# WilliamYi96/HGR-Net

Measured on AMD Instinct MI355X. Metric: images/sec over 21K-class hierarchy, batch 512; hit@1 parity vs reference, higher is better.
Workload: dtype f16

## Files before the change

hgr-net_amd/_lib.py:

```python
from __future__ import annotations

import ctypes as C
import os
from pathlib import Path

import torch

_HERE = Path(__file__).resolve().parent
LIB_PATH = Path(os.environ.get("HGR_LIB", _HERE / "lib" / "libhgr.so"))

HGR_BF16, HGR_F16 = 0, 1
EPI_NONE, EPI_BIAS, EPI_BIAS_QUICKGELU, EPI_BIAS_RESIDUAL, EPI_BIAS_RELU, EPI_BIAS_ADD16_RELU, EPI_ACCUM, EPI_QGELU_GRAD16 = 0, 1, 2, 3, 4, 5, 6, 7

_p, _i, _l, _f = C.c_void_p, C.c_int, C.c_int64, C.c_float

SIGNATURES = {
    "hgr_gemm_nt": [_p, _l, _p, _l, _p, _l, _p, _p, _l, _i, _i, _i, _i, _i, _i, _p],
    "hgr_gemm_set_tile": [_i],
    "hgr_gemm_set_tail": [_i, _i],
    "hgr_gemm_set_persist": [_i],
    "hgr_gemm_set_ws": [_i],
    "hgr_gemm_set_p8": [_i],
    "hgr_im2col_patches": [_p, _p, _i, _i, _i, _i, _i, _p],
    "hgr_im2col_patches_ex": [_p, _p, _i, _i, _i, _i, _i, _i, _i, _p],
# ... 52 lines not shown
    "hgr_avgpool2_bwd_nhwc": [_p, _p, _i, _i, _i, _i, _i, _p],
    "hgr_attnpool_tokens_bwd": [_p, _p, _i, _i, _i, _i, _p],
    "hgr_im2col3x3_t": [_p, _p, _i, _i, _i, _i, _l, _i, _p],
    "hgr_bn_fold": [_p, _p, _p, _p, _p, _f, _p, _p, _i, _i, _i, _i, _i, _p],
    "hgr_bn_unfold_grad": [_p, _l, _p, _p, _p, _p, _p, _f, _p, _p, _p, _i, _i, _i, _p],
    "hgr_csr_group_aggregate": [_p, _l, _p, _p, _p, _p, _i, _p, _p, _p, _p, _i, _p, _p, _p, _p, _i, _p, _p, _l, _i, _f, _i, _p],
    "hgr_gemm_nt_res_stats": [_p, _l, _p, _l, _p, _p, _l, _p, _p, _i, _i, _i, _i, _p],
    "hgr_vit_head": [_p, _p, _l, _l, _p, _p, _f, _p, _p, _i, _i, _i, _i, _p],
    "hgr_gemm_nt_res_stats_guard": [_p, _l, _p, _l, _p, _p, _l, _p, _p, _f, _p, _i, _i, _i, _i, _p],
    "hgr_gemm_nt_ln": [_p, _l, _p, _l, _p, _l, _p, _p, _p, _f, _i, _i, _i, _i, _i, _p],
    "hgr_gemm_nt_ln_mha": [_p, _l, _p, _l, _p, _p, _p, _f, _p, _l, _i, _i, _i, _i, _i, _p],
    "hgr_gemm_nt_bias_gelu_dual": [_p, _l, _p, _l, _p, _l, _p, _l, _p, _i, _i, _i, _i, _p],
    "hgr_gemm_nt_qgelu_grad_colsum": [_p, _l, _p, _l, _p, _l, _p, _l, _p, _i, _i, _i, _i, _p],
    "hgr_vit_embed_ln_stats": [_p, _p, _p, _p, _p, _p, _p, _p, _i, _i, _i, _f, _i, _p],
    "hgr_row_stats16": [_p, _p, _p, _p, _i, _i, _i, _p],
    "hgr_pair_rows_f32": [_p, _p, _p, _i, _i, _l, _p, _i, _p],
    "hgr_logits_eval_workspace_bytes": [_i, _i],
    "hgr_logits_eval": [_p, _p, _i, _i, _i, _p, _p, _p, _i, _p, _p, _i, _p, _i, _i, _p, _p, _p, _p, _i, _p],
    "hgr_logits_eval_tile_stage": [_p, _p, _i, _i, _i, _p, _p, _p, _i, _p, _p, _i, _p, _i, _i, _p, _p, _p, _p, _i, _p],
    "hgr_logits_eval_row_stage": [_p, _p, _i, _i, _i, _p, _p, _p, _i, _p, _p, _i, _p, _i, _i, _p, _p, _p, _p, _i, _p],
    "hgr_comm_unique_id": [_p],
    "hgr_comm_init": [_i, _i, _p],
    "hgr_comm_destroy": [],
    "hgr_comm_rank": [],
    "hgr_comm_world": [],
    "hgr_allreduce": [_p, _p, _l, _i, _i, _p],
    "hgr_allgather": [_p, _p, _l, _i, _p],
    "hgr_broadcast": [_p, _l, _i, _i, _p],
    "hgr_adamw": [_p, _p, _p, _p, _l, _f, _f, _f, _f, _f, _i, _p, _f, _f, _p],
}
# ... 55 lines not shown
```

hgr-net_amd/clip/model.py:

```python
from __future__ import annotations

import os
from collections import OrderedDict
from typing import Dict, Optional, Tuple, Union

import numpy as np
import torch
from torch import nn

from .. import ops
from .._lib import (EPI_BIAS, EPI_BIAS_ADD16_RELU, EPI_BIAS_QUICKGELU, EPI_BIAS_RELU, EPI_BIAS_RESIDUAL, EPI_NONE,
                    HgrError)


class QuickGELU(nn.Module):
    """Placeholder so ``mlp`` keeps the reference's child names (c_fc, gelu, c_proj); the activation
    itself is fused into the c_fc GEMM epilogue (HGR_EPI_BIAS_QUICKGELU)."""


class ResidualAttentionBlock(nn.Module):
    def __init__(self, d_model: int, n_head: int):
        super().__init__()
        self.attn = nn.MultiheadAttention(d_model, n_head)
        self.ln_1 = nn.LayerNorm(d_model)
# ... 111 lines not shown
        t = self._b.get("const." + name)
        if t is None:
            t = self._b["const." + name] = build()
            self.epoch += 1
        return t

    def get(self, name: str, shape, dtype, device) -> torch.Tensor:
        n = int(np.prod(shape))
        t = self._b.get(name)
        if t is None or t.numel() < n or t.dtype != dtype or t.device != device:
            t = torch.empty(n, dtype=dtype, device=device)
            self._b[name] = t
            self.epoch += 1
        return t[:n].view(*shape)


IMG_STREAMS = max(1, int(os.environ.get("HGR_IMG_STREAMS", "1")))
IMG_STREAMS_MIN_ROWS = 8192
CLS_LAST = os.environ.get("HGR_CLS_LAST", "1") != "0"
LN_FUSED = os.environ.get("HGR_LN_FUSED", "1") != "0"
QKV_MHA = os.environ.get("HGR_QKV_MHA", "1") != "0"


def ln_fusable(w: int, m: int = 0) -> bool:
    return LN_FUSED and w % 128 == 0 and m * 4 * w * 2 < 2 ** 32


def _run_blocks(x: Optional[torch.Tensor], blocks, heads: int, b: int, l: int, causal: bool, dt: torch.dtype, ws: _Workspace, tag: str,
                taps: Optional[dict] = None, tap_prefix: str = "", pair=None, stats: Optional[torch.Tensor] = None,
                flag: Optional[torch.Tensor] = None, cls_only_last: bool = False):
    m, w = (pair[0] if pair is not None else x).shape
    dev = (pair[0] if pair is not None else x).device
    qkv = ws.get(tag + ".qkv", (m, 3 * w), dt, dev)
    att = ws.get(tag + ".att", (m, w), dt, dev)
    u16 = ws.get(tag + ".u16", (m, 4 * w), dt, dev)
    if pair is not None:
        xh, xl = pair
        for i, k in enumerate(blocks):
            last_cls = cls_only_last and i == len(blocks) - 1 and l > 1 and 3 * w * l < (1 << 23)
            fused_attn = QKV_MHA and not last_cls and ops.ln_mha_ok(w, l, m, xh.stride(0))
            if last_cls:
                ch, cl = xh.view(b, l, w)[:, 0, :], xl.view(b, l, w)[:, 0, :]
                ops.gemm_nt_ln(xh, k.wf_in[w:], qkv[:, w:], k.s_in[w:], k.c_in[w:], stats, k.eps1, tag="kv")
                ops.split_point("class_token_tail")
                st_q = ws.get(tag + ".stats_q", (b, w // 64, 2), torch.float32, dev)
                idx = ws.const(f"cls_rows.{b}.{l}", lambda: (torch.arange(b, dtype=torch.int32, device=dev) * l).contiguous())
                ops.rows_gather(stats.view(b * l, -1), idx, st_q.view(b, -1))
                ops.gemm_nt_ln(ch, k.wf_in[:w], qkv.view(b, l, 3 * w)[:, 0, :w], k.s_in[:w], k.c_in[:w], st_q, k.eps1, tag="q_cls")
            elif fused_attn:
                ops.gemm_nt_ln_mha(xh, k.wf_in, att, k.s_in, k.c_in, stats, b, l, heads, causal, k.eps1)
            else:
                ops.gemm_nt_ln(xh, k.wf_in, qkv, k.s_in, k.c_in, stats, k.eps1, tag="qkv")
            if not fused_attn:
                ops.mha(qkv, att, b, l, heads, causal, q_rows=1 if last_cls else 0)
            if last_cls:
                ca = att.view(b, l, w)[:, 0, :]
                st_c = ws.get(tag + ".stats_cls", (b, w // 64, 2), torch.float32, dev)
                u_c = ws.get(tag + ".u16_cls", (b, 4 * w), dt, dev)
                ops.gemm_nt_res_stats(ca, k.w_out, ch, cl, k.b_out, st_c, tag="out_cls", flag=flag)
# ... 304 lines not shown
        return have[:n]

    def _vit_forward(self, image: torch.Tensor, p: dict, out: torch.Tensor, tag: str, taps: Optional[dict], u8: bool) -> bool:
        v = self.visual
        dt, ws, dev = self.image_dtype, self._ws, image.device
        b, r = image.shape[0], v.input_resolution
        ps = v.patch_size
        g = r // ps
        gg, l, w = g * g, g * g + 1, v.conv1.weight.shape[0]
        patches = ws.get(tag + ".patches", (b * gg, p["kp"]), dt, dev)
        if u8:
            ops.im2col_patches_u8(image, patches, ps)
        else:
            ops.im2col_patches(image, patches, ps)
        pe = ws.get(tag + ".pe", (b * gg, w), torch.float32, dev)
        ops.gemm_nt(patches, p["conv_w_nhwc"] if u8 else p["conv_w"], pe, tag="patch")
        cls16 = ws.get(tag + ".cls16", (b, w), dt, dev)
        fused = ln_fusable(w, b * l) and "v" not in self._ln_off
        if fused:
            xh = ws.get(tag + ".xh", (b * l, w), dt, dev)
            xl = ws.get(tag + ".xl", (b * l, w), ops.PAIR_LO, dev)
            stats = ws.get(tag + ".stats", (b * l, w // 64, 2), torch.float32, dev)
            ops.vit_embed_ln_stats(pe, p["cls"], p["pos"], p["ln_pre"][0], p["ln_pre"][1], xh, xl, stats, b, gg)
            if taps is not None:
                taps["visual.ln_pre"] = ops.pair_value(xh, xl).view(b, l, w)
            _run_blocks(None, p["vblocks"], w // 64, b, l, False, dt, ws, tag, taps, "visual.transformer", (xh, xl), stats, self._ln_flag("v", dev),
                        cls_only_last=taps is None and CLS_LAST)
            if w <= 1920 and w % 32 == 0 and v.output_dim % 4 == 0:
                ops.vit_head(xh, xl, l, p["ln_post"][0], p["ln_post"][1], float(v.ln_post.eps), p["proj_t"], out)
                return fused
            cls32 = ws.get(tag + ".cls32", (b, w), torch.float32, dev)
            ops.pair_rows_f32(xh, xl, cls32, row_mul=l)
            ops.layernorm(cls32, p["ln_post"][0], p["ln_post"][1], cls16, rows=b)
        else:
            x = ws.get(tag + ".x", (b * l, w), torch.float32, dev)
            ops.vit_embed_ln(pe, p["cls"], p["pos"], p["ln_pre"][0], p["ln_pre"][1], x, b, gg)
            if taps is not None:
                taps["visual.ln_pre"] = x.view(b, l, w).clone()
# ... 86 lines not shown
```

hgr-net_amd/csrc/hgr_common.h:

```cpp
#pragma once
#include <hip/hip_runtime.h>
#include <stdint.h>
#include <stdio.h>
#include <stdarg.h>
#include <stdlib.h>

#include "../../include/hgr.h"

#define HGR_WAVE 64

#ifdef HGR_LAB
#define HGR_LAB_ON(expr) (expr)
static inline int hgr_lab_env(const char *name) { const char *e = getenv(name); return e ? atoi(e) : 0; }
#else
#define HGR_LAB_ON(expr) false
static inline int hgr_lab_env(const char *) { return 0; }
#endif

typedef __attribute__((ext_vector_type(8))) __bf16 bf16x8;
typedef __attribute__((ext_vector_type(8))) _Float16 f16x8;
typedef __attribute__((ext_vector_type(4))) __bf16 bf16x4;
typedef __attribute__((ext_vector_type(4))) _Float16 f16x4;
typedef __attribute__((ext_vector_type(4))) float f32x4;
typedef __attribute__((ext_vector_type(16))) float f32x16;
// ... 126 lines not shown
}
__device__ __forceinline__ float wave_max(float v) {
#pragma unroll
    for (int o = 32; o > 0; o >>= 1) v = fmaxf(v, __shfl_xor(v, o));
    return v;
}

__device__ __forceinline__ float row16_sum(float v) {
    v += __builtin_bit_cast(float, __builtin_amdgcn_update_dpp(0, __builtin_bit_cast(int, v), 0xB1, 0xF, 0xF, true));
    v += __builtin_bit_cast(float, __builtin_amdgcn_update_dpp(0, __builtin_bit_cast(int, v), 0x4E, 0xF, 0xF, true));
    v += __builtin_bit_cast(float, __builtin_amdgcn_update_dpp(0, __builtin_bit_cast(int, v), 0x141, 0xF, 0xF, true));
    v += __builtin_bit_cast(float, __builtin_amdgcn_update_dpp(0, __builtin_bit_cast(int, v), 0x140, 0xF, 0xF, true));
    return v;
}

int hgr_set_error(int code, const char *fmt, ...);

#define HGR_REQUIRE(cond, ...)                                            \
    do {                                                                  \
        if (!(cond)) return hgr_set_error(HGR_EINVAL, __VA_ARGS__);       \
    } while (0)

#define HGR_CHECK_LAUNCH(name)                                                                      \
    do {                                                                                            \
        hipError_t e__ = hipGetLastError();                                                         \
        if (e__ != hipSuccess) return hgr_set_error(HGR_ELAUNCH, "%s: %s", name, hipGetErrorString(e__)); \
    } while (0)

static inline bool hgr_aligned(const void *p, size_t a) { return (reinterpret_cast<uintptr_t>(p) % a) == 0; }
```

hgr-net_amd/csrc/hgr_gemm.hip:

```cpp
#include "hgr_gemm_common.h"

using namespace hgr_gemm;

int hgr_conv3x3_c32_launch(const void *x, const void *w, const float *bias, void *out, int B, int H, int W, int Cout, int Kp,
                           int dtype, int relu, void *stream, int pool, int C);

namespace {
constexpr int BM = 128, BN = 128;

int duo_group_env() {
    static int g = -1;
    if (g < 0) { const char *e = getenv("HGR_GEMM_GROUP"); g = e ? atoi(e) : 0; if (g < 0) g = 0; }
    return g;
}
int duo_group() { return duo_group_env() ? duo_group_env() : 4; }
int duo_group_for(int tiles_n) { return duo_group_env() ? duo_group_env() : (tiles_n <= 8 ? 1 : 4); }
int duo_dbg() {
    static int d = -1;
    if (d < 0) d = hgr_lab_env("HGR_GEMM_DBG");
    return d;
}

struct DuoPlan { int big_panels, nbig, tiles_m_half, grid; };
int tail_env = -2, pb_env = -2;
// ... 180 lines not shown
        a.res = nullptr; a.ldr = 0; a.M = M; a.N = N; a.K = K;
        a.m_fastest = ((int64_t)N * K > (int64_t)M * K) ? 1 : 0;
        a.vec_ok = 1; a.dbg = dbg; a.kc = 0; a.csplit = 0; a.group = duo_group();
        launch_ws(a, dtype, WS_PLAIN, epilogue == HGR_EPI_BIAS_RELU ? 2 : 0, epilogue != HGR_EPI_NONE, s);
    }
    else if (duo_ok && (force == 2 || (force == 0 && tduo >= 256 && duo_fits))) launch_d();
    else if (force == 128 || K < 128) launch(0, M, false);
    else if (epi_has_idn16(epilogue) && force != 256) launch(0, M, false);
    else if (force == 256) launch(0, M, true);
    else if (cost_split < cost_big && cost_split < cost_small) { launch(0, m1, true); launch(m1, M - m1, false); }
    else launch(0, M, cost_big <= cost_small && t256 >= 128);
    HGR_CHECK_LAUNCH("hgr_gemm_nt");
    return HGR_OK;
}

static int conv3x3_launch(const void *x, const void *w, const float *bias, void *out,
                          int B, int H, int W, int C, int Cout, int stride, int Kp, int dtype, bool relu, void *stream) {
    HGR_REQUIRE(x && w && out && (bias || !relu), "hgr_conv3x3_nhwc: null operand");
    HGR_REQUIRE(B >= 1 && H >= 1 && W >= 1 && Cout >= 1 && (stride == 1 || stride == 2), "hgr_conv3x3_nhwc: bad geometry B=%d H=%d W=%d Cout=%d stride=%d", B, H, W, Cout, stride);
    HGR_REQUIRE(C >= 8 && C % 8 == 0 && C <= 16384, "hgr_conv3x3_nhwc: C=%d must be a multiple of 8 in [8, 16384]", C);
    HGR_REQUIRE(Kp >= 9 * C && Kp % BK == 0, "hgr_conv3x3_nhwc: Kp=%d must be >= 9*C and a multiple of %d", Kp, BK);
    HGR_REQUIRE(hgr_aligned(x, 16) && hgr_aligned(w, 16) && hgr_aligned(out, 8) && (!bias || hgr_aligned(bias, 16)) && Cout % 4 == 0, "hgr_conv3x3_nhwc: misaligned operand / Cout %% 4 != 0");
    HGR_REQUIRE(dtype == HGR_BF16 || dtype == HGR_F16, "hgr_conv3x3_nhwc: bad dtype %d", dtype);
    static int direct_env = -1;
    if (direct_env < 0) { const char *e = getenv("HGR_CONV_DIRECT"); direct_env = e ? atoi(e) : 1; }
    if (direct_env && C == 32 && stride == 1 && (Cout == 32 || Cout == 64) && Kp >= 288 && hgr_aligned(out, 16))
        return hgr_conv3x3_c32_launch(x, w, bias, out, B, H, W, Cout, Kp, dtype, relu ? 1 : 0, stream, 0, 32);
    if (direct_env && C == 64 && Cout == 64 && stride == 1 && Kp >= 576 && hgr_aligned(out, 16) && (int64_t)B * H * W >= 4096)
        return hgr_conv3x3_c32_launch(x, w, bias, out, B, H, W, Cout, Kp, dtype, relu ? 1 : 0, stream, 0, 64);
    const int Ho = (H + 2 - 3) / stride + 1, Wo = (W + 2 - 3) / stride + 1;
// ... 241 lines not shown
```

hgr-net_amd/csrc/hgr_gemm_common.h:

```cpp
#pragma once
#include "hgr_common.h"
#include <stdlib.h>
#include <type_traits>

namespace hgr_gemm {

constexpr int BK = 64;

struct GemmArgs {
    const char *A; int64_t lda;
    const char *W; int64_t ldw;
    void *C; int64_t ldc;
    const float *bias;
    const float *res; int64_t ldr;
    int M, N, K;
    int tiles_m, tiles_n;
    int m_fastest;
    int vec_ok;
    int dbg;
    int cH, cW, cC, cStride, cHo, cWo;
    unsigned cMagic;
    int cUni;
    int kc; int64_t csplit;
    float *ln_stats; int ln_slots; float ln_eps;
    void *ln_xh, *ln_xl; int64_t ln_ldx;
    const float *ln_s, *ln_c;
    unsigned *ln_flag; float ln_guard;
    int group;
    int nbig, big_panels, tiles_m_half;
    float *colsum = nullptr; int colsum_units = 0;
    int total = 0;
};


static __device__ __attribute__((aligned(16))) unsigned int hgr_zero_page[4] = {0u, 0u, 0u, 0u};

__device__ __forceinline__ float quick_gelu(float v) {
    return v * __builtin_amdgcn_rcpf(1.0f + __builtin_amdgcn_exp2f(-1.702f * 1.4426950408889634f * v));
}


template <int DT> __device__ __forceinline__ typename T16<DT>::elem quick_gelu16(float v) {
    return mul16<DT>(v, __builtin_amdgcn_rcpf(1.0f + __builtin_amdgcn_exp2f(-1.702f * 1.4426950408889634f * v)));
}
template <int DT> __device__ __forceinline__ typename T16<DT>::elem quick_gelu_train16(float x) {
// ... 224 lines not shown
```

hgr-net_amd/csrc/hgr_gemm_duo.hip:

```cpp
#include "hgr_gemm_common.h"

namespace hgr_gemm {

#ifndef HGR_PAIR_V2
#define HGR_PAIR_V2 1
#endif
constexpr int NTD = 256;
constexpr int DUO_A0 = 0, DUO_A1 = 32768, DUO_W0 = 65536, DUO_W1 = 73728, DUO_LDS = 81920;

__device__ __forceinline__ void store16_sc1(void *ptr, u32x4 v) {
    asm volatile("global_store_dwordx4 %0, %1, off sc1\n\ts_nop 1" ::"v"(ptr), "v"(v) : "memory");
}

template <int DT, int EPI, bool OUT32, int LN, int MH, bool CONV = false>
__device__ __forceinline__ void duo_tile(const GemmArgs &p, char *smem, const int m0, const int n0) {
    typedef typename T16<DT>::vec8 vec8;
    typedef typename T16<DT>::elem E;
    constexpr int WR = 64 * MH;
    int tid = threadIdx.x;
    if (LN == 1) asm volatile("" : "+v"(tid));
    const int lane = tid & 63;
    const int wave = __builtin_amdgcn_readfirstlane(tid >> 6);
    const int wm = wave >> 1, wn = wave & 1;
    const int r = lane & 15, g = lane >> 4;
// ... 786 lines not shown
    for (int a = 0; a < MH; ++a)
#pragma unroll
    for (int i = 0; i < 4; ++i) {
        const int m = m0 + wm * WR + a * 64 + i * 16 + r;
        if (m >= p.M) continue;
#pragma unroll
        for (int b = 0; b < 2; ++b)
#pragma unroll
        for (int j = 0; j < 2; ++j) {
            const int n = n0 + wn * 64 + b * 32 + j * 16 + g * 4;
            if (n < p.N) store_quad<DT, EPI, OUT32>(p, acc[a][b][i][j], m, n);
        }
    }
}

template <int DT, int EPI, bool OUT32, int LN = 0, bool CONV = false>
__global__ __launch_bounds__(NTD, 2) void gemm_nt_duo(GemmArgs p) {
    if (p.kc) {
        const int sp = blockIdx.y;
        p.A += (int64_t)sp * p.kc * 2; p.W += (int64_t)sp * p.kc * 2;
        p.C = (char *)p.C + (int64_t)sp * p.csplit * 4;
        p.K = min(p.kc, p.K - sp * p.kc);
    }
    __shared__ __attribute__((aligned(1024))) char smem[DUO_LDS];
    constexpr bool PERSIST = LN == 1;
    const int total = PERSIST && p.total > 0 ? p.total : (int)gridDim.x;
  auto one_tile = [&](const int vb) {
    const bool half = vb >= p.nbig;
    const int nwg = half ? total - p.nbig : p.nbig;
    const int orig = half ? vb - p.nbig : vb;
// ... 1 lines not shown
    const int xcd = orig & 7, q8 = nwg >> 3, r8 = nwg & 7;
    const int wg = (xcd < r8 ? xcd * (q8 + 1) : r8 * (q8 + 1) + (xcd - r8) * q8) + (orig >> 3);
    const int GROUP = p.group;
    int tm, tn;
    if (p.m_fastest) {
        const int per = GROUP * tiles_m, grp = wg / per, first = grp * GROUP;
        const int gs = min(GROUP, p.tiles_n - first), loc = wg - grp * per;
        tn = first + loc % gs; tm = loc / gs;
    } else {
        const int per = GROUP * p.tiles_n, grp = wg / per, first = grp * GROUP;
        const int gs = min(GROUP, tiles_m - first), loc = wg - grp * per;
        tm = first + loc % gs; tn = loc / gs;
    }
    if (half) duo_tile<DT, EPI, OUT32, LN, 1, CONV>(p, smem, p.big_panels * 256 + tm * 128, tn * 128);
    else duo_tile<DT, EPI, OUT32, LN, 2, CONV>(p, smem, tm * 256, tn * 128);
  };
    if constexpr (PERSIST) {
        for (int vb = (int)blockIdx.x; vb < total; vb += (int)gridDim.x) {
            one_tile(vb);
            if (vb + (int)gridDim.x < total) HGR_RBAR();
        }
    } else one_tile((int)blockIdx.x);
}

namespace {
template <int DT>
void launch_duo_dt(const GemmArgs &a, int epi, bool out32, int ln, dim3 grid, hipStream_t s) {
    switch (ln) {
        case 1: hipLaunchKernelGGL((gemm_nt_duo<DT, HGR_EPI_BIAS_RESIDUAL, true, 1>), grid, dim3(NTD), 0, s, a); return;
        case 2:
            if (epi == HGR_EPI_BIAS_QUICKGELU) hipLaunchKernelGGL((gemm_nt_duo<DT, HGR_EPI_BIAS_QUICKGELU, false, 2>), grid, dim3(NTD), 0, s, a);
            else hipLaunchKernelGGL((gemm_nt_duo<DT, HGR_EPI_BIAS, false, 2>), grid, dim3(NTD), 0, s, a);
            return;
        case 4: hipLaunchKernelGGL((gemm_nt_duo<DT, HGR_EPI_BIAS, false, 4>), grid, dim3(NTD), 0, s, a); return;
        case 5: hipLaunchKernelGGL((gemm_nt_duo<DT, HGR_EPI_BIAS_RELU, false, 0, true>), grid, dim3(NTD), 0, s, a); return;
        default: break;
    }
#define HGR_DUO(E) do { if (out32) hipLaunchKernelGGL((gemm_nt_duo<DT, E, true>), grid, dim3(NTD), 0, s, a); \
                        else hipLaunchKernelGGL((gemm_nt_duo<DT, E, false>), grid, dim3(NTD), 0, s, a); } while (0)
    switch (epi) {
        case HGR_EPI_NONE: HGR_DUO(HGR_EPI_NONE); break;
        case HGR_EPI_BIAS: HGR_DUO(HGR_EPI_BIAS); break;
        case HGR_EPI_BIAS_QUICKGELU: HGR_DUO(HGR_EPI_BIAS_QUICKGELU); break;
        case HGR_EPI_BIAS_RELU: HGR_DUO(HGR_EPI_BIAS_RELU); break;
        case HGR_EPI_BIAS_ADD16_RELU: hipLaunchKernelGGL((gemm_nt_duo<DT, HGR_EPI_BIAS_ADD16_RELU, false>), grid, dim3(NTD), 0, s, a); break;
        case HGR_EPI_ACCUM: hipLaunchKernelGGL((gemm_nt_duo<DT, HGR_EPI_ACCUM, true>), grid, dim3(NTD), 0, s, a); break;
        case HGR_EPI_QGELU_GRAD16: hipLaunchKernelGGL((gemm_nt_duo<DT, HGR_EPI_QGELU_GRAD16, false>), grid, dim3(NTD), 0, s, a); break;
        default: hipLaunchKernelGGL((gemm_nt_duo<DT, HGR_EPI_BIAS_RESIDUAL, true>), grid, dim3(NTD), 0, s, a); break;
// ... 34 lines not shown
```

hgr-net_amd/csrc/hgr_norm.hip:

```cpp
#include "hgr_common.h"

namespace {

constexpr int MAXV = 16;

template <int DT, bool OUT32, int NV>
__global__ __launch_bounds__(256) void layernorm_rows(const float *__restrict__ x, const float *__restrict__ gamma,
                                                      const float *__restrict__ beta, void *__restrict__ y,
                                                      int rows, int W, int64_t row_mul, const int32_t *__restrict__ row_idx, float eps) {
    const int lane = threadIdx.x & 63;
    const int row = blockIdx.x * 4 + (threadIdx.x >> 6);
    if (row >= rows) return;
    const int64_t src = (int64_t)row * row_mul + (row_idx ? row_idx[row] : 0);
    const f32x4 *xr = (const f32x4 *)(x + src * W);
    const int nv = W >> 2;
    f32x4 v[NV];
    float s = 0.f;
#pragma unroll
    for (int i = 0; i < NV; ++i) {
        const int c = i * 64 + lane;
        if (i * 64 < nv) {
            v[i] = (c < nv) ? xr[c] : (f32x4){0.f, 0.f, 0.f, 0.f};
            s += v[i][0] + v[i][1] + v[i][2] + v[i][3];
        }
// ... 25 lines not shown
}

template <int NV, int DT = HGR_F16, bool STATS = false>
__global__ __launch_bounds__(256) void vit_embed_ln(const float *__restrict__ patches, const float *__restrict__ cls,
                                                    const float *__restrict__ pos, const float *__restrict__ gamma,
                                                    const float *__restrict__ beta, float *__restrict__ x,
                                                    int B, int G, int W, float eps, void *__restrict__ xh = nullptr, void *__restrict__ xl = nullptr,
                                                    float *__restrict__ stats = nullptr) {
    const int lane = threadIdx.x & 63;
    const int L = G + 1;
    const int row = blockIdx.x * 4 + (threadIdx.x >> 6);
    if (row >= B * L) return;
    const int b = row / L, t = row - b * L;
    const f32x4 *src = (const f32x4 *)(t == 0 ? cls : patches + ((int64_t)b * G + (t - 1)) * W);
    const f32x4 *pr = (const f32x4 *)(pos + (int64_t)t * W);
    const int nv = W >> 2;
    f32x4 v[NV];
    float s = 0.f;
#pragma unroll
    for (int i = 0; i < NV; ++i) {
        const int c = i * 64 + lane;
        if (i * 64 < nv) {
            v[i] = (c < nv) ? (src[c] + pr[c]) : (f32x4){0.f, 0.f, 0.f, 0.f};
            s += v[i][0] + v[i][1] + v[i][2] + v[i][3];
        }
    }
    const float mean = wave_sum(s) / (float)W;
    float q = 0.f;
#pragma unroll
    for (int i = 0; i < NV; ++i) {
        const int c = i * 64 + lane;
        if (i * 64 < nv && c < nv) {
#pragma unroll
            for (int e = 0; e < 4; ++e) { const float d = v[i][e] - mean; q += d * d; }
        }
    }
    const float rstd = rsqrtf(wave_sum(q) / (float)W + eps);
    const f32x4 *gv = (const f32x4 *)gamma, *bv = (const f32x4 *)beta;
    f32x4 *out = STATS ? nullptr : (f32x4 *)(x + (int64_t)row * W);
#pragma unroll
    for (int i = 0; i < NV; ++i) {
        const int c = i * 64 + lane;
        if (i * 64 < nv && c < nv) {
            const f32x4 ga = gv[c], be = bv[c];
            f32x4 o;
#pragma unroll
            for (int e = 0; e < 4; ++e) o[e] = (v[i][e] - mean) * rstd * ga[e] + be[e];
            if (!STATS) out[c] = o;
            if (STATS) {
                typename T16<DT>::vec4 nh;
                unsigned nl = 0u;
#pragma unroll
                for (int e = 0; e < 4; ++e) { unsigned q; typename T16<DT>::elem h; pair_split<DT>(o[e], h, q); nh[e] = h; nl |= q << (8 * e); }
                ((typename T16<DT>::vec4 *)((typename T16<DT>::elem *)xh + (int64_t)row * W))[c] = nh;
                ((unsigned *)((unsigned char *)xl + (int64_t)row * W))[c] = nl;
                const float s1 = row16_sum((o[0] + o[1]) + (o[2] + o[3]));
                const float s2 = row16_sum((o[0] * o[0] + o[1] * o[1]) + (o[2] * o[2] + o[3] * o[3]));
                if ((lane & 15) == 0) *(float2 *)(stats + ((int64_t)row * (W >> 6) + (c >> 4)) * 2) = make_float2(s1, s2);
            }
        }
    }
}

template <int DT>
__global__ __launch_bounds__(256) void row_stats16(const float *__restrict__ x, void *__restrict__ xh, void *__restrict__ xl, float *__restrict__ stats, int rows, int W) {
    const int lane = threadIdx.x & 63;
    const int row = blockIdx.x * 4 + (threadIdx.x >> 6);
    if (row >= rows) return;
    const f32x4 *xr = (const f32x4 *)(x + (int64_t)row * W);
    const int nv = W >> 2;
    for (int c0 = 0; c0 < nv; c0 += 64) {
        const int c = c0 + lane;
        const bool ok = c < nv;
        const f32x4 v = ok ? xr[c] : (f32x4){0.f, 0.f, 0.f, 0.f};
        const float s1 = row16_sum((v[0] + v[1]) + (v[2] + v[3]));
        const float s2 = row16_sum((v[0] * v[0] + v[1] * v[1]) + (v[2] * v[2] + v[3] * v[3]));
// ... 271 lines not shown
```

hgr-net_amd/model/clip_tree.py:

```python
from __future__ import annotations

import copy
import math
import os
import random
from typing import Optional, Sequence

import torch
import torch.nn as nn

from .. import clip, ops
from ..hierarchy import build_hierarchy
from .._lib import HgrError

TEMPLATE = "a photo of a {}."

TAIL_OVERLAP = os.environ.get("HGR_TAIL_OVERLAP", "1") != "0"
LOGITS_SPLIT = os.environ.get("HGR_LOGITS_SPLIT", "class")


class _StopHead(Exception):
    """Raised by the split hook while the HEAD graph of a pipelined step is captured: the rest of the step belongs to the tail graph."""


# ... 174 lines not shown

    @torch.no_grad()
    def forward_eval_overlapped(self, inputs, plan, k: int, consume) -> bool:
        if not (TAIL_OVERLAP and self.use_graph and inputs.is_cuda) or self._zsl16 is None:
            return False
        if inputs.dtype not in (torch.float32, torch.uint8) or not inputs.is_contiguous():
            return False
        from ..clip import model as _clip_model
        if _clip_model.IMG_STREAMS > 1:
            return False
        plan.bind(self._eval_class_operand(), self._zsl16.shape[1])
        mode = ("eval", plan, k)
        st = self._pipe_state(inputs.device)
        self.clip_model.poll_ln_guard()
        gen = (tuple(inputs.shape), inputs.dtype, self._zsl16.data_ptr(), self.clip_model._fingerprint(), tuple(sorted(self.clip_model._ln_off)),
               id(plan), plan.zsl.data_ptr(), k)
        main = torch.cuda.current_stream()
        if gen != st["gen"]:
            main.wait_stream(st["side"])
            st["graphs"].clear()
            st["static"].clear()
            st["misses"] = 0
            ok = True
            for tag in ("v", "v@1"):
                ok &= self._eager_phase(inputs, mode, "head", tag)[1]
                if ok:
                    self._eager_phase(inputs, mode, "tail", tag)
            main.synchronize()
            st["gen"], st["ok"] = gen, ok
        if not st["ok"]:
            return False
# ... 168 lines not shown
```

hgr-net_amd/ops.py:

```python
from __future__ import annotations

from typing import Optional

import torch

from . import _lib
from ._lib import (EPI_ACCUM, EPI_BIAS, EPI_BIAS_ADD16_RELU, EPI_BIAS_QUICKGELU, EPI_BIAS_RELU, EPI_BIAS_RESIDUAL, EPI_NONE, EPI_QGELU_GRAD16,
                   HGR_BF16, HGR_F16)

PROFILE = None

WEIGHTS_GEN = [0]

SPLIT_HOOK = None


def split_point(name: str) -> None:
    h = SPLIT_HOOK
    if h is not None:
        h(name)


TORCH16 = {HGR_BF16: torch.bfloat16, HGR_F16: torch.float16}
PAIR_LO = torch.uint8
# ... 131 lines not shown
    _prof_end(ev, 2.0 * m * 3 * w * k + 4.0 * b * heads * l * l * 64, 2 * m * k + 2 * 3 * w * k + 2 * m * w, tag)
    return att


def ln_mha_ok(w: int, l: int, rows: Optional[int] = None, ldx: Optional[int] = None) -> bool:
    if not (1 <= l <= 64 and w % 128 == 0):
        return False
    if rows is not None and rows * (ldx if ldx is not None else w) * 2 >= (1 << 32):
        return False
    return 3 * w * w * 2 < (1 << 32)


def vit_embed_ln_stats(patches, cls, pos, gamma, beta, xh, xl, stats, b, g, eps=1e-5):
    _lib.call("hgr_vit_embed_ln_stats", _dev(patches), _dev(cls), _dev(pos), _dev(gamma), _dev(beta), _dev(xh), _dev(xl), _dev(stats),
              b, g, xh.shape[1], eps, DT_OF[xh.dtype], _stream())


def row_stats16(x: torch.Tensor, xh: torch.Tensor, xl: torch.Tensor, stats: torch.Tensor) -> None:
    assert x.dtype == torch.float32 and x.is_contiguous() and xh.is_contiguous() and xl.is_contiguous() and xh.shape == xl.shape == x.shape
    assert xl.dtype == PAIR_LO and stats.numel() >= x.shape[0] * (x.shape[1] // 64) * 2
    _lib.call("hgr_row_stats16", _dev(x), _dev(xh), _dev(xl), _dev(stats), x.shape[0], x.shape[1], DT_OF[xh.dtype], _stream())


def pair_rows_f32(xh: torch.Tensor, xl: torch.Tensor, out: torch.Tensor, row_mul: int = 1, row_idx: Optional[torch.Tensor] = None) -> torch.Tensor:
    assert xh.is_contiguous() and xl.is_contiguous() and out.is_contiguous() and out.dtype == torch.float32 and out.shape[1] == xh.shape[1] and xl.dtype == PAIR_LO
    _lib.call("hgr_pair_rows_f32", _dev(xh), _dev(xl), _dev(out), out.shape[0], out.shape[1], row_mul, _dev(row_idx), DT_OF[xh.dtype], _stream())
    return out


def vit_head(xh: torch.Tensor, xl: torch.Tensor, row_mul: int, gamma: torch.Tensor, beta: torch.Tensor, eps: float, proj_t: torch.Tensor,
# ... 611 lines not shown
```

include/hgr.h:

```cpp
#ifndef HGR_H
#define HGR_H

#include <stdint.h>

#ifdef __cplusplus
extern "C" {
#endif

#define HGR_ABI_VERSION 4

enum { HGR_OK = 0, HGR_EINVAL = -1, HGR_EUNSUPPORTED = -2, HGR_ELAUNCH = -3 };

typedef enum { HGR_BF16 = 0, HGR_F16 = 1 } hgr_dtype_t;

typedef enum {
    HGR_EPI_NONE = 0,
    HGR_EPI_BIAS = 1,
    HGR_EPI_BIAS_QUICKGELU = 2,
    HGR_EPI_BIAS_RESIDUAL = 3,
    HGR_EPI_BIAS_RELU = 4,
    HGR_EPI_BIAS_ADD16_RELU = 5,
    HGR_EPI_ACCUM = 6,
    HGR_EPI_QGELU_GRAD16 = 7
} hgr_epilogue_t;
// ... 173 lines not shown
int hgr_gemm_nt_ln(const void *XH, int64_t ldx, const void *Wfold, int64_t ldw, void *C, int64_t ldc,
                   const float *ln_s, const float *ln_c, const float *stats, float eps,
                   int M, int N, int K, int dtype, int act, void *stream);

int hgr_gemm_nt_ln_mha(const void *XH, int64_t ldx, const void *Wfold, int64_t ldw, const float *ln_s, const float *ln_c,
                       const float *stats, float eps, void *att, int64_t ldatt, int B, int L, int heads, int causal,
                       int dtype, void *stream);

int hgr_gemm_nt_bias_gelu_dual(const void *A, int64_t lda, const void *W, int64_t ldw, void *pre, int64_t ldpre, void *post, int64_t ldpost,
                               const float *bias, int M, int N, int K, int dtype, void *stream);
int hgr_gemm_nt_qgelu_grad_colsum(const void *A, int64_t lda, const void *W, int64_t ldw, void *C, int64_t ldc, const void *pre, int64_t ldpre,
                                  float *colsum_part, int M, int N, int K, int dtype, void *stream);
int hgr_vit_embed_ln_stats(const float *patches, const float *class_embedding, const float *positional_embedding,
                           const float *gamma, const float *beta, void *xh, void *xl, float *stats,
                           int B, int G, int W, float eps, int dtype, void *stream);
int hgr_row_stats16(const float *x, void *xh, void *xl, float *stats, int rows, int W, int dtype, void *stream);
int hgr_pair_rows_f32(const void *xh, const void *xl, float *out, int rows, int W, int64_t row_mul, const int32_t *row_idx, int dtype, void *stream);

int64_t hgr_logits_eval_workspace_bytes(int rows, int n_perm);
int hgr_logits_eval(const void *feat16, const void *zsl_perm16, int rows, int D, int n_perm,
                    const int32_t *tpos_perm, const int32_t *epos_perm, const int32_t *level_first,
                    int n_levels, const int32_t *filler_pos, const int32_t *train_cols, int n_train,
                    const int32_t *test_cols, int n_test, int k,
                    int32_t *out_level, int32_t *out_top1, int32_t *out_topk, void *workspace, int dtype, void *stream);
int hgr_logits_eval_tile_stage(const void *feat16, const void *zsl_perm16, int rows, int D, int n_perm,
                    const int32_t *tpos_perm, const int32_t *epos_perm, const int32_t *level_first,
                    int n_levels, const int32_t *filler_pos, const int32_t *train_cols, int n_train,
                    const int32_t *test_cols, int n_test, int k,
                    int32_t *out_level, int32_t *out_top1, int32_t *out_topk, void *workspace, int dtype, void *stream);
int hgr_logits_eval_row_stage(const void *feat16, const void *zsl_perm16, int rows, int D, int n_perm,
// ... 23 lines not shown
```

Measured before the change: 107,200.

## Fuse patch-embedding GEMM with embed+ln_pre via last-arriving-tile counters

Result: slower. 105,500 (-1.6%).

```diff
diff --git a/hgr-net_amd/_lib.py b/hgr-net_amd/_lib.py
--- a/hgr-net_amd/_lib.py
+++ b/hgr-net_amd/_lib.py
@@ -90,6 +90,7 @@
     "hgr_gemm_nt_qgelu_grad_colsum": [_p, _l, _p, _l, _p, _l, _p, _l, _p, _i, _i, _i, _i, _p],
     "hgr_vit_embed_ln_stats": [_p, _p, _p, _p, _p, _p, _p, _p, _i, _i, _i, _f, _i, _p],
     "hgr_row_stats16": [_p, _p, _p, _p, _i, _i, _i, _p],
+    "hgr_gemm_nt_patch_embed": [_p, _l, _p, _l, _p, _l, _p, _p, _p, _p, _p, _p, _p, _p, _i, _i, _i, _i, _i, _f, _i, _p],
     "hgr_pair_rows_f32": [_p, _p, _p, _i, _i, _l, _p, _i, _p],
     "hgr_logits_eval_workspace_bytes": [_i, _i],
     "hgr_logits_eval": [_p, _p, _i, _i, _i, _p, _p, _p, _i, _p, _p, _i, _p, _i, _i, _p, _p, _p, _p, _i, _p],
diff --git a/hgr-net_amd/clip/model.py b/hgr-net_amd/clip/model.py
--- a/hgr-net_amd/clip/model.py
+++ b/hgr-net_amd/clip/model.py
@@ -149,12 +149,23 @@
             self.epoch += 1
         return t[:n].view(*shape)
 
+    def zeros(self, name: str, shape, dtype, device) -> torch.Tensor:
+        n = int(np.prod(shape))
+        t = self._b.get(name)
+        if t is None or t.numel() < n or t.dtype != dtype or t.device != device:
+            t = torch.zeros(n, dtype=dtype, device=device)
+            self._b[name] = t
+            self.epoch += 1
+        return t[:n].view(*shape)
+
 
 IMG_STREAMS = max(1, int(os.environ.get("HGR_IMG_STREAMS", "1")))
 IMG_STREAMS_MIN_ROWS = 8192
 CLS_LAST = os.environ.get("HGR_CLS_LAST", "1") != "0"
 LN_FUSED = os.environ.get("HGR_LN_FUSED", "1") != "0"
 QKV_MHA = os.environ.get("HGR_QKV_MHA", "1") != "0"
+PATCH_FUSED = os.environ.get("HGR_PATCH_FUSED", "1") != "0"
+KV_IN_TAIL = os.environ.get("HGR_KV_IN_TAIL", "1") != "0"
 
 
 def ln_fusable(w: int, m: int = 0) -> bool:
@@ -176,8 +187,11 @@
             fused_attn = QKV_MHA and not last_cls and ops.ln_mha_ok(w, l, m, xh.stride(0))
             if last_cls:
                 ch, cl = xh.view(b, l, w)[:, 0, :], xl.view(b, l, w)[:, 0, :]
+                if KV_IN_TAIL:
+                    ops.split_point("class_token_tail")
                 ops.gemm_nt_ln(xh, k.wf_in[w:], qkv[:, w:], k.s_in[w:], k.c_in[w:], stats, k.eps1, tag="kv")
-                ops.split_point("class_token_tail")
+                if not KV_IN_TAIL:
+                    ops.split_point("class_token_tail")
                 st_q = ws.get(tag + ".stats_q", (b, w // 64, 2), torch.float32, dev)
                 idx = ws.const(f"cls_rows.{b}.{l}", lambda: (torch.arange(b, dtype=torch.int32, device=dev) * l).contiguous())
                 ops.rows_gather(stats.view(b * l, -1), idx, st_q.view(b, -1))
@@ -512,14 +526,21 @@
         else:
             ops.im2col_patches(image, patches, ps)
         pe = ws.get(tag + ".pe", (b * gg, w), torch.float32, dev)
-        ops.gemm_nt(patches, p["conv_w_nhwc"] if u8 else p["conv_w"], pe, tag="patch")
+        wconv = p["conv_w_nhwc"] if u8 else p["conv_w"]
         cls16 = ws.get(tag + ".cls16", (b, w), dt, dev)
         fused = ln_fusable(w, b * l) and "v" not in self._ln_off
+        one_launch = fused and PATCH_FUSED and ops.patch_embed_ok(b * gg, w, patches.shape[1], patches.stride(0), wconv.stride(0))
+        if not one_launch:
+            ops.gemm_nt(patches, wconv, pe, tag="patch")
         if fused:
             xh = ws.get(tag + ".xh", (b * l, w), dt, dev)
             xl = ws.get(tag + ".xl", (b * l, w), ops.PAIR_LO, dev)
             stats = ws.get(tag + ".stats", (b * l, w // 64, 2), torch.float32, dev)
-            ops.vit_embed_ln_stats(pe, p["cls"], p["pos"], p["ln_pre"][0], p["ln_pre"][1], xh, xl, stats, b, gg)
+            if one_launch:
+                cnt = ws.zeros(tag + ".pe_cnt", ((b * gg + 127) // 128,), torch.int32, dev)
+                ops.gemm_nt_patch_embed(patches, wconv, pe, p["cls"], p["pos"], p["ln_pre"][0], p["ln_pre"][1], xh, xl, stats, cnt, b, gg)
+            else:
+                ops.vit_embed_ln_stats(pe, p["cls"], p["pos"], p["ln_pre"][0], p["ln_pre"][1], xh, xl, stats, b, gg)
             if taps is not None:
                 taps["visual.ln_pre"] = ops.pair_value(xh, xl).view(b, l, w)
             _run_blocks(None, p["vblocks"], w // 64, b, l, False, dt, ws, tag, taps, "visual.transformer", (xh, xl), stats, self._ln_flag("v", dev),
diff --git a/hgr-net_amd/csrc/hgr_common.h b/hgr-net_amd/csrc/hgr_common.h
--- a/hgr-net_amd/csrc/hgr_common.h
+++ b/hgr-net_amd/csrc/hgr_common.h
@@ -164,6 +164,68 @@
     return v;
 }
 
+template <int NV>
+__device__ __forceinline__ void vit_embed_row_load(const f32x4 *src, const f32x4 *pr, int W, int lane, f32x4 (&v)[NV]) {
+    const int nv = W >> 2;
+#pragma unroll
+    for (int i = 0; i < NV; ++i) {
+        const int c = i * 64 + lane;
+        if (i * 64 < nv) v[i] = (c < nv) ? (src[c] + pr[c]) : (f32x4){0.f, 0.f, 0.f, 0.f};
+    }
+}
+template <int NV, int DT, bool STATS>
+__device__ __forceinline__ void vit_embed_row_finish(const f32x4 (&v)[NV], const float *gamma, const float *beta, int W, float eps, int lane,
+                                                     float *x32, void *xh_row, void *xl_row, float *stats_row) {
+    const int nv = W >> 2;
+    float s = 0.f;
+#pragma unroll
+    for (int i = 0; i < NV; ++i) {
+        if (i * 64 < nv) s += v[i][0] + v[i][1] + v[i][2] + v[i][3];
+    }
+    const float mean = wave_sum(s) / (float)W;
+    float q = 0.f;
+#pragma unroll
+    for (int i = 0; i < NV; ++i) {
+        const int c = i * 64 + lane;
+        if (i * 64 < nv && c < nv) {
+#pragma unroll
+            for (int e = 0; e < 4; ++e) { const float d = v[i][e] - mean; q += d * d; }
+        }
+    }
+    const float rstd = rsqrtf(wave_sum(q) / (float)W + eps);
+    const f32x4 *gv = (const f32x4 *)gamma, *bv = (const f32x4 *)beta;
+    f32x4 *out = (f32x4 *)x32;
+#pragma unroll
+    for (int i = 0; i < NV; ++i) {
+        const int c = i * 64 + lane;
+        if (i * 64 < nv && c < nv) {
+            const f32x4 ga = gv[c], be = bv[c];
+            f32x4 o;
+#pragma unroll
+            for (int e = 0; e < 4; ++e) o[e] = (v[i][e] - mean) * rstd * ga[e] + be[e];
+            if (!STATS) out[c] = o;
+            if (STATS) {
+                typename T16<DT>::vec4 nh;
+                unsigned nl = 0u;
+#pragma unroll
+                for (int e = 0; e < 4; ++e) { unsigned q8; typename T16<DT>::elem h; pair_split<DT>(o[e], h, q8); nh[e] = h; nl |= q8 << (8 * e); }
+                ((typename T16<DT>::vec4 *)xh_row)[c] = nh;
+                ((unsigned *)xl_row)[c] = nl;
+                const float s1 = row16_sum((o[0] + o[1]) + (o[2] + o[3]));
+                const float s2 = row16_sum((o[0] * o[0] + o[1] * o[1]) + (o[2] * o[2] + o[3] * o[3]));
+                if ((lane & 15) == 0) *(float2 *)(stats_row + (c >> 4) * 2) = make_float2(s1, s2);
+            }
+        }
+    }
+}
+template <int NV, int DT, bool STATS>
+__device__ __forceinline__ void vit_embed_row(const f32x4 *src, const f32x4 *pr, const float *gamma, const float *beta, int W, float eps,
+                                              int lane, float *x32, void *xh_row, void *xl_row, float *stats_row) {
+    f32x4 v[NV];
+    vit_embed_row_load<NV>(src, pr, W, lane, v);
+    vit_embed_row_finish<NV, DT, STATS>(v, gamma, beta, W, eps, lane, x32, xh_row, xl_row, stats_row);
+}
+
 int hgr_set_error(int code, const char *fmt, ...);
 
 #define HGR_REQUIRE(cond, ...)                                            \
diff --git a/hgr-net_amd/csrc/hgr_gemm.hip b/hgr-net_amd/csrc/hgr_gemm.hip
--- a/hgr-net_amd/csrc/hgr_gemm.hip
+++ b/hgr-net_amd/csrc/hgr_gemm.hip
@@ -218,6 +218,39 @@
     return HGR_OK;
 }
 
+extern "C" int hgr_gemm_nt_patch_embed(const void *A, int64_t lda, const void *W, int64_t ldw, float *pe, int64_t ldpe,
+                                       const float *class_embedding, const float *positional_embedding, const float *gamma, const float *beta,
+                                       void *xh, void *xl, float *stats, uint32_t *counters, int n_counters,
+                                       int B, int G, int N, int K, float eps, int dtype, void *stream) {
+    HGR_REQUIRE(A && W && pe && class_embedding && positional_embedding && gamma && beta && xh && xl && stats && counters, "hgr_gemm_nt_patch_embed: null operand");
+    HGR_REQUIRE(B >= 1 && G >= 1 && (int64_t)B * G < (1ll << 31) && (int64_t)B * (G + 1) < (1ll << 31), "hgr_gemm_nt_patch_embed: B=%d G=%d unsupported", B, G);
+    const int M = B * G;
+    HGR_REQUIRE(N >= 64 && N % 64 == 0 && N <= 1024, "hgr_gemm_nt_patch_embed: N=%d unsupported (a multiple of 64, at most 1024)", N);
+    HGR_REQUIRE(K >= 128 && K % BK == 0, "hgr_gemm_nt_patch_embed: K=%d must be a multiple of %d and >= 128 (pad the operands)", K, BK);
+    HGR_REQUIRE(lda >= K && ldw >= K && lda % 8 == 0 && ldw % 8 == 0, "hgr_gemm_nt_patch_embed: lda=%lld ldw=%lld must be >= K and multiples of 8", (long long)lda, (long long)ldw);
+    HGR_REQUIRE(ldpe >= N && ldpe % 4 == 0 && ldpe < (1 << 20), "hgr_gemm_nt_patch_embed: ldpe=%lld must be >= N, a multiple of 4 and < 2^20", (long long)ldpe);
+    HGR_REQUIRE((int64_t)M * lda * 2 < (1ll << 32) && (int64_t)N * ldw * 2 < (1ll << 32), "hgr_gemm_nt_patch_embed: operands must stay below 4 GB (32-bit offsets)");
+    HGR_REQUIRE(hgr_aligned(A, 16) && hgr_aligned(W, 16) && hgr_aligned(pe, 16) && hgr_aligned(class_embedding, 16) && hgr_aligned(positional_embedding, 16) &&
+                hgr_aligned(gamma, 16) && hgr_aligned(beta, 16) && hgr_aligned(xh, 8) && hgr_aligned(xl, 8) && hgr_aligned(stats, 8) && hgr_aligned(counters, 4),
+                "hgr_gemm_nt_patch_embed: misaligned operand");
+    HGR_REQUIRE(n_counters >= (M + 127) / 128, "hgr_gemm_nt_patch_embed: %d counters, %d needed (one per 128 patch rows)", n_counters, (M + 127) / 128);
+    HGR_REQUIRE(dtype == HGR_BF16 || dtype == HGR_F16, "hgr_gemm_nt_patch_embed: bad dtype %d", dtype);
+    GemmArgs a;
+    a.A = (const char *)A; a.lda = lda; a.W = (const char *)W; a.ldw = ldw; a.C = pe; a.ldc = ldpe; a.bias = nullptr;
+    a.res = nullptr; a.ldr = 0; a.M = M; a.N = N; a.K = K;
+    a.tiles_m = (M + 255) / 256; a.tiles_n = (N + 127) / 128;
+    a.m_fastest = ((int64_t)N * K > (int64_t)M * K) ? 1 : 0;
+    a.vec_ok = 1; a.dbg = duo_dbg(); a.kc = 0; a.csplit = 0; a.group = duo_group();
+    a.ln_stats = stats; a.ln_slots = N / 64; a.ln_eps = eps; a.ln_xh = xh; a.ln_xl = xl; a.ln_ldx = N;
+    a.ln_s = nullptr; a.ln_c = nullptr; a.ln_flag = nullptr; a.ln_guard = 0.f;
+    a.emb_cls = class_embedding; a.emb_pos = positional_embedding; a.emb_gamma = gamma; a.emb_beta = beta; a.emb_cnt = counters; a.emb_G = G;
+    dim3 grid;
+    duo_apply_plan(a, true, grid);
+    launch_duo(a, dtype, HGR_EPI_NONE, true, 3, grid, (hipStream_t)stream);
+    HGR_CHECK_LAUNCH("hgr_gemm_nt_patch_embed");
+    return HGR_OK;
+}
+
 static int conv3x3_launch(const void *x, const void *w, const float *bias, void *out,
                           int B, int H, int W, int C, int Cout, int stride, int Kp, int dtype, bool relu, void *stream) {
     HGR_REQUIRE(x && w && out && (bias || !relu), "hgr_conv3x3_nhwc: null operand");
diff --git a/hgr-net_amd/csrc/hgr_gemm_common.h b/hgr-net_amd/csrc/hgr_gemm_common.h
--- a/hgr-net_amd/csrc/hgr_gemm_common.h
+++ b/hgr-net_amd/csrc/hgr_gemm_common.h
@@ -29,6 +29,8 @@
     int group;
     int nbig, big_panels, tiles_m_half;
     float *colsum = nullptr; int colsum_units = 0;
+    const float *emb_cls = nullptr, *emb_pos = nullptr, *emb_gamma = nullptr, *emb_beta = nullptr;
+    unsigned *emb_cnt = nullptr; int emb_G = 0;
     int total = 0;
 };
 
diff --git a/hgr-net_amd/csrc/hgr_gemm_duo.hip b/hgr-net_amd/csrc/hgr_gemm_duo.hip
--- a/hgr-net_amd/csrc/hgr_gemm_duo.hip
+++ b/hgr-net_amd/csrc/hgr_gemm_duo.hip
@@ -824,6 +824,72 @@
     }
 }
 
+template <int DT>
+__device__ __forceinline__ void duo_embed_arrive(const GemmArgs &p, char *smem, const int unit, const int m0, const int mrows) {
+    typedef typename T16<DT>::elem E;
+    asm volatile("s_waitcnt vmcnt(0)" ::: "memory");
+    __syncthreads();
+    unsigned *const last = (unsigned *)smem;
+    if (threadIdx.x == 0) {
+        __builtin_amdgcn_fence(__ATOMIC_RELEASE, "agent");
+        asm volatile("s_waitcnt vmcnt(0)" ::: "memory");
+        const unsigned old = __hip_atomic_fetch_add(p.emb_cnt + unit, 1u, __ATOMIC_RELAXED, __HIP_MEMORY_SCOPE_AGENT);
+        const bool mine = old == (unsigned)(p.tiles_n - 1);
+        if (mine) {
+            __builtin_amdgcn_fence(__ATOMIC_ACQUIRE, "agent");
+            asm volatile("s_waitcnt vmcnt(0)" ::: "memory");
+            __hip_atomic_store(p.emb_cnt + unit, 0u, __ATOMIC_RELAXED, __HIP_MEMORY_SCOPE_AGENT);
+        }
+        *last = mine ? 1u : 0u;
+    }
+    __syncthreads();
+    if (!*last) return;
+    const int lane = threadIdx.x & 63, wave = threadIdx.x >> 6;
+    const int G = p.emb_G, L = G + 1, W = p.N;
+    const int nvl = (W / 4 + 63) / 64;
+    auto rows = [&](auto nv_tag) {
+        constexpr int NV = decltype(nv_tag)::value;
+        constexpr int R = 4;
+        const int nj = mrows > wave ? (mrows - wave + 3) / 4 : 0;
+        auto load = [&](f32x4 (&v)[R][NV], const int j0) {
+#pragma unroll
+            for (int r = 0; r < R; ++r) {
+                const int gm = m0 + wave + 4 * min(j0 + r, nj - 1);
+                const int t = gm % G;
+                vit_embed_row_load<NV>((const f32x4 *)((const float *)p.C + (int64_t)gm * p.ldc), (const f32x4 *)(p.emb_pos + (int64_t)(t + 1) * W), W, lane, v[r]);
+            }
+        };
+        auto finish = [&](const f32x4 (&v)[R][NV], const int j0) {
+#pragma unroll
+            for (int r = 0; r < R; ++r) {
+                if (j0 + r >= nj) break;
+                const int gm = m0 + wave + 4 * (j0 + r);
+                const int64_t row = (int64_t)(gm / G) * L + 1 + gm % G;
+                vit_embed_row_finish<NV, DT, true>(v[r], p.emb_gamma, p.emb_beta, W, p.ln_eps, lane, nullptr, (E *)p.ln_xh + row * W,
+                                                   (unsigned char *)p.ln_xl + row * W, p.ln_stats + row * (W >> 6) * 2);
+            }
+        };
+        f32x4 va[R][NV], vb[R][NV];
+        if (nj > 0) load(va, 0);
+        for (int j0 = 0; j0 < nj; j0 += 2 * R) {
+            if (j0 + R < nj) load(vb, j0 + R);
+            finish(va, j0);
+            if (j0 + R < nj) {
+                if (j0 + 2 * R < nj) load(va, j0 + 2 * R);
+                finish(vb, j0 + R);
+            }
+        }
+        for (int b = (m0 + G - 1) / G + wave; b <= (m0 + mrows - 1) / G; b += 4) {
+            const int64_t row = (int64_t)b * L;
+            vit_embed_row<NV, DT, true>((const f32x4 *)p.emb_cls, (const f32x4 *)p.emb_pos, p.emb_gamma, p.emb_beta, W, p.ln_eps, lane, nullptr,
+                                        (E *)p.ln_xh + row * W, (unsigned char *)p.ln_xl + row * W, p.ln_stats + row * (W >> 6) * 2);
+        }
+    };
+    if (nvl <= 1) rows(std::integral_constant<int, 1>());
+    else if (nvl <= 2) rows(std::integral_constant<int, 2>());
+    else rows(std::integral_constant<int, 4>());
+}
+
 template <int DT, int EPI, bool OUT32, int LN = 0, bool CONV = false>
 __global__ __launch_bounds__(NTD, 2) void gemm_nt_duo(GemmArgs p) {
     if (p.kc) {
@@ -855,6 +921,10 @@
     }
     if (half) duo_tile<DT, EPI, OUT32, LN, 1, CONV>(p, smem, p.big_panels * 256 + tm * 128, tn * 128);
     else duo_tile<DT, EPI, OUT32, LN, 2, CONV>(p, smem, tm * 256, tn * 128);
+    if constexpr (LN == 3) {
+        const int m0 = half ? p.big_panels * 256 + tm * 128 : tm * 256;
+        duo_embed_arrive<DT>(p, smem, half ? p.big_panels + tm : tm, m0, min(half ? 128 : 256, p.M - m0));
+    }
   };
     if constexpr (PERSIST) {
         for (int vb = (int)blockIdx.x; vb < total; vb += (int)gridDim.x) {
@@ -873,6 +943,7 @@
             if (epi == HGR_EPI_BIAS_QUICKGELU) hipLaunchKernelGGL((gemm_nt_duo<DT, HGR_EPI_BIAS_QUICKGELU, false, 2>), grid, dim3(NTD), 0, s, a);
             else hipLaunchKernelGGL((gemm_nt_duo<DT, HGR_EPI_BIAS, false, 2>), grid, dim3(NTD), 0, s, a);
             return;
+        case 3: hipLaunchKernelGGL((gemm_nt_duo<DT, HGR_EPI_NONE, true, 3>), grid, dim3(NTD), 0, s, a); return;
         case 4: hipLaunchKernelGGL((gemm_nt_duo<DT, HGR_EPI_BIAS, false, 4>), grid, dim3(NTD), 0, s, a); return;
         case 5: hipLaunchKernelGGL((gemm_nt_duo<DT, HGR_EPI_BIAS_RELU, false, 0, true>), grid, dim3(NTD), 0, s, a); return;
         default: break;
diff --git a/hgr-net_amd/csrc/hgr_norm.hip b/hgr-net_amd/csrc/hgr_norm.hip
--- a/hgr-net_amd/csrc/hgr_norm.hip
+++ b/hgr-net_amd/csrc/hgr_norm.hip
@@ -63,52 +63,10 @@
     const int b = row / L, t = row - b * L;
     const f32x4 *src = (const f32x4 *)(t == 0 ? cls : patches + ((int64_t)b * G + (t - 1)) * W);
     const f32x4 *pr = (const f32x4 *)(pos + (int64_t)t * W);
-    const int nv = W >> 2;
-    f32x4 v[NV];
-    float s = 0.f;
-#pragma unroll
-    for (int i = 0; i < NV; ++i) {
-        const int c = i * 64 + lane;
-        if (i * 64 < nv) {
-            v[i] = (c < nv) ? (src[c] + pr[c]) : (f32x4){0.f, 0.f, 0.f, 0.f};
-            s += v[i][0] + v[i][1] + v[i][2] + v[i][3];
-        }
-    }
-    const float mean = wave_sum(s) / (float)W;
-    float q = 0.f;
-#pragma unroll
-    for (int i = 0; i < NV; ++i) {
-        const int c = i * 64 + lane;
-        if (i * 64 < nv && c < nv) {
-#pragma unroll
-            for (int e = 0; e < 4; ++e) { const float d = v[i][e] - mean; q += d * d; }
-        }
-    }
-    const float rstd = rsqrtf(wave_sum(q) / (float)W + eps);
-    const f32x4 *gv = (const f32x4 *)gamma, *bv = (const f32x4 *)beta;
-    f32x4 *out = STATS ? nullptr : (f32x4 *)(x + (int64_t)row * W);
-#pragma unroll
-    for (int i = 0; i < NV; ++i) {
-        const int c = i * 64 + lane;
-        if (i * 64 < nv && c < nv) {
-            const f32x4 ga = gv[c], be = bv[c];
-            f32x4 o;
-#pragma unroll
-            for (int e = 0; e < 4; ++e) o[e] = (v[i][e] - mean) * rstd * ga[e] + be[e];
-            if (!STATS) out[c] = o;
-            if (STATS) {
-                typename T16<DT>::vec4 nh;
-                unsigned nl = 0u;
-#pragma unroll
-                for (int e = 0; e < 4; ++e) { unsigned q; typename T16<DT>::elem h; pair_split<DT>(o[e], h, q); nh[e] = h; nl |= q << (8 * e); }
-                ((typename T16<DT>::vec4 *)((typename T16<DT>::elem *)xh + (int64_t)row * W))[c] = nh;
-                ((unsigned *)((unsigned char *)xl + (int64_t)row * W))[c] = nl;
-                const float s1 = row16_sum((o[0] + o[1]) + (o[2] + o[3]));
-                const float s2 = row16_sum((o[0] * o[0] + o[1] * o[1]) + (o[2] * o[2] + o[3] * o[3]));
-                if ((lane & 15) == 0) *(float2 *)(stats + ((int64_t)row * (W >> 6) + (c >> 4)) * 2) = make_float2(s1, s2);
-            }
-        }
-    }
+    typedef typename T16<DT>::elem E;
+    vit_embed_row<NV, DT, STATS>(src, pr, gamma, beta, W, eps, lane, STATS ? nullptr : x + (int64_t)row * W,
+                                 STATS ? (void *)((E *)xh + (int64_t)row * W) : nullptr, STATS ? (void *)((unsigned char *)xl + (int64_t)row * W) : nullptr,
+                                 STATS ? stats + (int64_t)row * (W >> 6) * 2 : nullptr);
 }
 
 template <int DT>
diff --git a/hgr-net_amd/model/clip_tree.py b/hgr-net_amd/model/clip_tree.py
--- a/hgr-net_amd/model/clip_tree.py
+++ b/hgr-net_amd/model/clip_tree.py
@@ -212,7 +212,7 @@
         st = self._pipe_state(inputs.device)
         self.clip_model.poll_ln_guard()
         gen = (tuple(inputs.shape), inputs.dtype, self._zsl16.data_ptr(), self.clip_model._fingerprint(), tuple(sorted(self.clip_model._ln_off)),
-               id(plan), plan.zsl.data_ptr(), k)
+               id(plan), plan.zsl.data_ptr(), k, _clip_model.KV_IN_TAIL, _clip_model.PATCH_FUSED)
         main = torch.cuda.current_stream()
         if gen != st["gen"]:
             main.wait_stream(st["side"])
diff --git a/hgr-net_amd/ops.py b/hgr-net_amd/ops.py
--- a/hgr-net_amd/ops.py
+++ b/hgr-net_amd/ops.py
@@ -169,6 +169,24 @@
 def vit_embed_ln_stats(patches, cls, pos, gamma, beta, xh, xl, stats, b, g, eps=1e-5):
     _lib.call("hgr_vit_embed_ln_stats", _dev(patches), _dev(cls), _dev(pos), _dev(gamma), _dev(beta), _dev(xh), _dev(xl), _dev(stats),
               b, g, xh.shape[1], eps, DT_OF[xh.dtype], _stream())
+
+
+def patch_embed_ok(m: int, n: int, k: int, lda: int, ldw: int) -> bool:
+    return n % 64 == 0 and 64 <= n <= 1024 and k % 64 == 0 and k >= 128 and m * lda * 2 < (1 << 32) and n * ldw * 2 < (1 << 32)
+
+
+def gemm_nt_patch_embed(a: torch.Tensor, w: torch.Tensor, pe: torch.Tensor, cls, pos, gamma, beta, xh: torch.Tensor, xl: torch.Tensor,
+                        stats: torch.Tensor, counters: torch.Tensor, b: int, g: int, eps: float = 1e-5, tag: str = "patch") -> None:
+    m, k = a.shape
+    n = w.shape[0]
+    assert m == b * g and w.shape[1] == k and a.dtype == w.dtype == xh.dtype and a.stride(1) == w.stride(1) == pe.stride(1) == 1
+    assert pe.dtype == torch.float32 and pe.shape == (m, n) and xl.dtype == PAIR_LO and xh.shape == xl.shape == (b * (g + 1), n)
+    assert xh.is_contiguous() and xl.is_contiguous() and stats.dtype == torch.float32 and stats.numel() >= b * (g + 1) * (n // 64) * 2
+    assert counters.element_size() == 4 and counters.is_contiguous()
+    ev = _prof_begin()
+    _lib.call("hgr_gemm_nt_patch_embed", _dev(a), a.stride(0), _dev(w), w.stride(0), _dev(pe), pe.stride(0), _dev(cls), _dev(pos), _dev(gamma), _dev(beta),
+              _dev(xh), _dev(xl), _dev(stats), _dev(counters), counters.numel(), b, g, n, k, float(eps), DT_OF[a.dtype], _stream())
+    _prof_end(ev, 2.0 * m * n * k, 2 * m * k + 2 * n * k + 4 * m * n, tag)
 
 
 def row_stats16(x: torch.Tensor, xh: torch.Tensor, xl: torch.Tensor, stats: torch.Tensor) -> None:
diff --git a/include/hgr.h b/include/hgr.h
--- a/include/hgr.h
+++ b/include/hgr.h
@@ -211,6 +211,10 @@
 int hgr_vit_embed_ln_stats(const float *patches, const float *class_embedding, const float *positional_embedding,
                            const float *gamma, const float *beta, void *xh, void *xl, float *stats,
                            int B, int G, int W, float eps, int dtype, void *stream);
+int hgr_gemm_nt_patch_embed(const void *A, int64_t lda, const void *W, int64_t ldw, float *pe, int64_t ldpe,
+                            const float *class_embedding, const float *positional_embedding, const float *gamma, const float *beta,
+                            void *xh, void *xl, float *stats, uint32_t *counters, int n_counters,
+                            int B, int G, int N, int K, float eps, int dtype, void *stream);
 int hgr_row_stats16(const float *x, void *xh, void *xl, float *stats, int rows, int W, int dtype, void *stream);
 int hgr_pair_rows_f32(const void *xh, const void *xl, float *out, int rows, int W, int64_t row_mul, const int32_t *row_idx, int dtype, void *stream);
 
```
